# anon-aadhaar/anon-aadhaar-halo2

Hardware: AMD Instinct MI355X
Metric: create_proof wall-clock (ms) + proofs/sec, full Aadhaar circuit, 1/2/4/8 GPU (higher is better)
Workload: dtype u32 limbs (254-bit Montgomery integers: 9 x 29-bit in the hot products, 8 x 32-bit elsewhere)

## Files before the change

### anon-aadhaar-halo2_amd/csrc/msm.hip

```cpp
#include <stdlib.h>
#include <string.h>

#include "common.hpp"
#include "fp29.cuh"
#include "fp29_quad.cuh"

using namespace bn254;

struct amdzk_srs {
  uint32_t k = 0;
  uint32_t c = 0;
  uint32_t W = 0;
  size_t n = 0;
  G1Affine* table[AMDZK_NUM_BASES] = {nullptr, nullptr, nullptr};
  G1Affine* base[AMDZK_NUM_BASES] = {nullptr, nullptr, nullptr};
  std::mutex prefix_guard;
  double prefix_build_ms = 0;
};
static size_t srs_basis_bytes(const amdzk_srs* s) { return ((size_t)s->W + 1) * s->n * sizeof(G1Affine); }

uint32_t zk_srs_k(const amdzk_srs* srs) { return srs->k; }
bool zk_srs_has_basis(const amdzk_srs* srs, int basis) { return srs && basis >= 0 && basis < AMDZK_NUM_BASES && srs->table[basis]; }

namespace {
// ... 1305 lines not shown
  ZK_LAUNCH(ctx, "msm_blk_offsets", msm_blk_offsets_kernel, dim3((nb + 255) / 256, (unsigned)ncols), dim3(256), 0, blk_hist, cnt, nb, g.nblk);
  ZK_LAUNCH(ctx, "msm_scan", msm_scan_kernel, dim3((unsigned)ncols), dim3(1024), scan_shmem, cnt, off[0], nb, 1u, 1);
  if (per_window) ZK_TRY(launch_digits_win<true>(ctx, g.c, da, dgrid));
  else if (d_col_ptrs) ZK_TRY((launch_digits<true, true>(ctx, g.c, da, dgrid, g.big_digits)));
  else ZK_TRY((launch_digits<true, false>(ctx, g.c, da, dgrid, g.big_digits)));
  for (int l = 1; l <= MSM_NLEV; l++) {
    const uint32_t T = l == 1 ? g.T1 : g.TL;
    ZK_LAUNCH(ctx, "msm_scan", msm_scan_kernel, dim3((unsigned)ncols), dim3(1024), scan_shmem, off[l - 1], off[l], nb, T, 2);
    AccArgs a;
    a.off_in = off[l - 1];
    a.off_out = off[l];
    a.nb = nb;
    a.T = T;
    a.entries = entries;
    a.ecap = g.ecap;
    a.table = table;
    a.in_list = list[l - 1];
    a.in_cap = g.cap[l - 1];
    a.out_list = list[l];
    a.out_cap = g.cap[l];
    const size_t threads = (g.cap[l - 1] + T - 1) / T;
    dim3 grid((unsigned)((threads + MSM_THREADS - 1) / MSM_THREADS), (unsigned)ncols);
    if (l == 1) {
      ZK_LAUNCH(ctx, "msm_accum_l1", msm_accum_seg_kernel<true>, grid, dim3(MSM_THREADS), 0, a);
      ZK_HIP(ctx, hipEventRecord(l1_done, ctx->stream));
    } else if (quad_on && !(getenv("AMDZK_FOLD_QUAD") && atoi(getenv("AMDZK_FOLD_QUAD")) == 0)) {
      const dim3 qgrid((unsigned)((4 * threads + MSM_THREADS - 1) / MSM_THREADS), (unsigned)ncols);
      ZK_LAUNCH(ctx, "msm_accum_fold", msm_accum_fold_quad_kernel, qgrid, dim3(MSM_THREADS), 0, a);
    } else {
      ZK_LAUNCH(ctx, "msm_accum_fold", msm_accum_seg_kernel<false>, grid, dim3(MSM_THREADS), 0, a);
    }
  }
  const unsigned fold_w = (unsigned)((g.G + 63) / 64);
  ZK_LAUNCH(ctx, "msm_accum_final", msm_accum_final_kernel, dim3(nb / 64, (unsigned)ncols), dim3(64), 0, off[MSM_NLEV], nb, list[MSM_NLEV],
            g.cap[MSM_NLEV], dense);
  static const int tail_tree = getenv("AMDZK_TAIL_TREE") ? atoi(getenv("AMDZK_TAIL_TREE")) : -1;
  const bool quad = quad_on && fold_w == 1;
  if (quad)
    ZK_LAUNCH(ctx, "msm_rowcol", msm_rowcol_quad_kernel, dim3(64, 2, (unsigned)ncols), dim3(256), 0, dense, nb, rows, cols);
  else if ((tail_tree < 0 ? g.latency : tail_tree != 0) && ncols <= 65535)
    ZK_LAUNCH(ctx, "msm_rowcol", msm_rowcol_tree_kernel, dim3(64, (unsigned)(2 * ((g.G + 63) / 64)), (unsigned)ncols), dim3(64), 0, dense, nb, rows, cols);
  else
    ZK_LAUNCH(ctx, "msm_rowcol", msm_rowcol_kernel, dim3((unsigned)(2 * ((g.G + 63) / 64)), (unsigned)ncols), dim3(64 * ROWCOL_WAVES), 0, dense, nb, rows, cols);
  if (quad) ZK_LAUNCH(ctx, "msm_fold", msm_fold_quad_kernel, dim3((unsigned)ncols), dim3(512), 0, rows, cols, nb, outp);
  else if (fold_w == 1) ZK_LAUNCH(ctx, "msm_fold", msm_fold_kernel<1>, dim3((unsigned)ncols), dim3(128), 0, rows, cols, nb, outp);
  else ZK_LAUNCH(ctx, "msm_fold", msm_fold_kernel<8>, dim3((unsigned)ncols), dim3(64 * (fold_w + 1)), 0, rows, cols, nb, outp);
  return AMDZK_OK;
}

static int msm_check_basis(amdzk_ctx* ctx, const amdzk_srs* srs, int basis) {
  if (!srs || basis < 0 || basis >= AMDZK_NUM_BASES) ZK_FAIL(ctx, AMDZK_E_INVALID, "msm: no parameters or basis %d unknown", basis);
  if (srs->table[basis]) return AMDZK_OK;
  if (basis == AMDZK_BASIS_G_LAGRANGE_PREFIX)
    ZK_FAIL(ctx, AMDZK_E_INVALID, "msm: the prefix-sum basis has not been built (it is made with the first proving key that has permutation columns)");
  ZK_FAIL(ctx, AMDZK_E_INVALID, "msm: basis %d not uploaded", basis);
}

int zk_msm_dev_xyzz(amdzk_ctx* ctx, const amdzk_srs* srs, int basis, const Fr* d_scalars, size_t ncols,
                    size_t len, size_t col_stride, G1X** d_out) {
  ZK_TRY(msm_check_basis(ctx, srs, basis));
  if (len > srs->n) ZK_FAIL(ctx, AMDZK_E_INVALID, "msm: len %zu > 2^k = %zu", len, srs->n);
  if (ncols == 0 || ncols > 65535) ZK_FAIL(ctx, AMDZK_E_INVALID, "msm: ncols %zu out of range", ncols);
  if ((uint64_t)srs->W * srs->n >= (1ull << 31)) ZK_FAIL(ctx, AMDZK_E_UNSUPPORTED, "msm: table too large for 31-bit ids");
  const MsmGeom g = msm_geometry(srs, ncols, len, ctx->msm_latency_mode);
  const size_t o_out = align_up(g.bytes, 256);
  char* ws = nullptr;
  ZK_TRY(zk_ws_reserve(ctx, 1, o_out + align_up(ncols * sizeof(G1X), 256), (void**)&ws));
  G1X* outp = (G1X*)(ws + o_out);
  if (!ctx->msm_l1_evt) ZK_HIP(ctx, hipEventCreateWithFlags(&ctx->msm_l1_evt, hipEventDisableTiming));
  ZK_TRY(msm_group(ctx, srs->table[basis], (uint32_t)srs->n, false, g, ws, d_scalars, ncols, len, col_stride, outp, ctx->msm_l1_evt));
  ctx->msm_l1_fresh = true;
  *d_out = outp;
  return AMDZK_OK;
}

static constexpr size_t MSM_COLS_WS_BYTES = (size_t)16 << 30;
int zk_msm_dev_xyzz_cols(amdzk_ctx* ctx, const amdzk_srs* srs, int basis, const Fr* const* d_col_ptrs, size_t ncols, size_t len,
                         size_t max_ws_bytes, G1X** d_out) {
  ZK_TRY(msm_check_basis(ctx, srs, basis));
  if (len > srs->n) ZK_FAIL(ctx, AMDZK_E_INVALID, "msm: len %zu > 2^k = %zu", len, srs->n);
  if (!d_col_ptrs || ncols == 0) ZK_FAIL(ctx, AMDZK_E_INVALID, "msm: no column pointer table or ncols == 0");
  if ((uint64_t)srs->W * srs->n >= (1ull << 31)) ZK_FAIL(ctx, AMDZK_E_UNSUPPORTED, "msm: table too large for 31-bit ids");
  const size_t cap = max_ws_bytes ? max_ws_bytes : MSM_COLS_WS_BYTES;
  size_t runs = (ncols + 65534) / 65535, per = 0, bytes = 0;
  for (;; runs++) {
    per = (ncols + runs - 1) / runs;
    const size_t last = ncols - (ncols - 1) / per * per;
    bytes = std::max(msm_geometry(srs, per, len, ctx->msm_latency_mode).bytes, msm_geometry(srs, last, len, ctx->msm_latency_mode).bytes);
    if (per == 1 || bytes <= cap) break;
  }
  const size_t o_scratch = align_up(ncols * sizeof(G1X), 256);
  char* ws = nullptr;
  ZK_TRY(zk_ws_reserve(ctx, 1, o_scratch + align_up(bytes, 256), (void**)&ws));
  G1X* outp = (G1X*)ws;
  if (!ctx->msm_l1_evt) ZK_HIP(ctx, hipEventCreateWithFlags(&ctx->msm_l1_evt, hipEventDisableTiming));
  for (size_t first = 0; first < ncols; first += per) {
    const size_t cnt = std::min(per, ncols - first);
    const MsmGeom gr = msm_geometry(srs, cnt, len, ctx->msm_latency_mode);
    ZK_TRY(msm_group(ctx, srs->table[basis], (uint32_t)srs->n, false, gr, ws + o_scratch, nullptr, cnt, len, 0, outp + first, ctx->msm_l1_evt,
                     d_col_ptrs + first));
  }
  ctx->msm_l1_fresh = true;
  *d_out = outp;
  return AMDZK_OK;
}

static uint32_t pick_window_bits_bases(size_t len) {
// ... 103 lines not shown
```

### anon-aadhaar-halo2_amd/csrc/plonk_kernels.hip

```cpp
#include <stdlib.h>
#include <string.h>

#include "plonk_kernels.hpp"
#include "fp29.cuh"

using namespace bn254;

namespace {

__device__ __forceinline__ Fr ld_fr(const Fr* p) {
  const uint4* q = reinterpret_cast<const uint4*>(p);
  uint4 a = q[0], b = q[1];
  Fr r;
  r.l[0] = a.x; r.l[1] = a.y; r.l[2] = a.z; r.l[3] = a.w;
  r.l[4] = b.x; r.l[5] = b.y; r.l[6] = b.z; r.l[7] = b.w;
  return r;
}
__device__ __forceinline__ void st_fr(Fr* p, const Fr& v) {
  uint4* q = reinterpret_cast<uint4*>(p);
  q[0] = make_uint4(v.l[0], v.l[1], v.l[2], v.l[3]);
  q[1] = make_uint4(v.l[4], v.l[5], v.l[6], v.l[7]);
}

__device__ __forceinline__ bool op_reads_col(uint32_t op) {
// ... 297 lines not shown
__global__ __launch_bounds__(256) void batch_invert_kernel(Fr* a, Fr* scratch, size_t total) {
  __shared__ Fr pre[256], suf[256];
  const uint32_t t = threadIdx.x;
  const size_t base = (size_t)blockIdx.x * 256 * BI_E + t;
  Fr acc = Fr::one();
#pragma unroll 1
  for (uint32_t j = 0; j < BI_E; j++) {
    const size_t i = base + (size_t)j * 256;
    if (i >= total) break;
    st_fr(scratch + i, acc);
    const Fr v = ld_fr(a + i);
    if (!v.is_zero()) acc = fr29_mul_std(acc, v);
  }
  pre[t] = acc;
  suf[t] = acc;
  __syncthreads();
  for (uint32_t d = 1; d < 256; d <<= 1) {
    const Fr p = t >= d ? pre[t - d] : Fr::one();
    const Fr q = t + d < 256 ? suf[t + d] : Fr::one();
    __syncthreads();
    if (t >= d) pre[t] = fr29_mul_std(p, pre[t]);
    if (t + d < 256) suf[t] = fr29_mul_std(suf[t], q);
    __syncthreads();
  }
  __shared__ Fr tot_inv;
  if (t == 0) tot_inv = inv_gcd(pre[255]);
  __syncthreads();
  acc = tot_inv;
  if (t > 0) acc = fr29_mul_std(acc, pre[t - 1]);
  if (t < 255) acc = fr29_mul_std(acc, suf[t + 1]);
#pragma unroll 1
  for (uint32_t j = BI_E; j-- > 0;) {
    const size_t i = base + (size_t)j * 256;
    if (i >= total) continue;
    const Fr v = ld_fr(a + i);
    if (v.is_zero()) continue;
    st_fr(a + i, fr29_mul_std(acc, ld_fr(scratch + i)));
    acc = fr29_mul_std(acc, v);
  }
}

__global__ __launch_bounds__(256) void mul_elem_kernel(Fr* a, const Fr* b, size_t total) {
  for (size_t i = (size_t)blockIdx.x * blockDim.x + threadIdx.x; i < total; i += (size_t)gridDim.x * blockDim.x)
    st_fr(a + i, fr29_mul_std(ld_fr(a + i), ld_fr(b + i)));
}

__global__ __launch_bounds__(256) void row_diff_kernel(const Fr* z, Fr* d, size_t n, size_t z_stride, size_t d_stride) {
  const size_t i = (size_t)blockIdx.x * blockDim.x + threadIdx.x;
  if (i >= n) return;
  const Fr* zc = z + (size_t)blockIdx.y * z_stride;
  Fr v = ld_fr(zc + i);
  if (i + 1 < n) v = sub(v, ld_fr(zc + i + 1));
  st_fr(d + (size_t)blockIdx.y * d_stride + i, v);
}

constexpr int SCAN_E = 8;
constexpr int SCAN_BLOCK = 256 * SCAN_E;

__global__ __launch_bounds__(256) void scan_local_kernel(const Fr* in, Fr* out, Fr* totals, size_t n, size_t col_stride,
                                                         uint32_t nblk) {
  __shared__ Fr part[256];
  const uint32_t col = blockIdx.y, blk = blockIdx.x, t = threadIdx.x;
  const Fr* src = in + (size_t)col * col_stride;
  Fr* dst = out + (size_t)col * col_stride;
  const size_t base = (size_t)blk * SCAN_BLOCK + (size_t)t * SCAN_E;
  Fr tot = Fr::one();
#pragma unroll 1
  for (int i = 0; i < SCAN_E; i++)
    if (base + i < n) tot = i == 0 ? ld_fr(src + base) : fr29_mul_std(tot, ld_fr(src + base + i));
  part[t] = tot;
  __syncthreads();
  for (uint32_t d = 1; d < 256; d <<= 1) {
    Fr v = t >= d ? part[t - d] : Fr::one();
    __syncthreads();
    if (t >= d) part[t] = fr29_mul_std(v, part[t]);
    __syncthreads();
  }
  Fr pre = t == 0 ? Fr::one() : part[t - 1];
#pragma unroll 1
  for (int i = 0; i < SCAN_E; i++) {
    if (base + i >= n) break;
    const Fr v = ld_fr(src + base + i);
    st_fr(dst + base + i, pre);
    pre = fr29_mul_std(pre, v);
  }
  if (t == 255) st_fr(totals + (size_t)col * nblk + blk, part[255]);
}

__global__ void scan_blocks_kernel(Fr* totals, const Fr* local, Fr* rel, uint32_t ncols, uint32_t nblk, size_t col_stride,
                                   size_t u) {
  const uint32_t col = blockIdx.x * blockDim.x + threadIdx.x;
  if (col >= ncols) return;
  Fr* t = totals + (size_t)col * nblk;
  Fr acc = Fr::one();
  for (uint32_t b = 0; b < nblk; b++) {
    Fr v = ld_fr(t + b);
    st_fr(t + b, acc);
    acc = fr29_mul_std(acc, v);
  }
  if (rel) st_fr(rel + col, fr29_mul_std(ld_fr(t + u / SCAN_BLOCK), ld_fr(local + (size_t)col * col_stride + u)));
}

__global__ void scan_chain_kernel(const Fr* rel, Fr* start, uint32_t ncols) {
  if (blockIdx.x != 0 || threadIdx.x != 0) return;
  Fr acc = Fr::one();
  for (uint32_t c = 0; c < ncols; c++) {
// ... 400 lines not shown
  for (uint32_t p = 1; p < nparts; p++) acc = add(acc, ld_fr(h + (size_t)p * rows + row));
  st_fr(h + row, acc);
}

int zk_expr_eval_limbs(amdzk_ctx* ctx, const ExprArgs& a, uint32_t depth, const char* name) {
  size_t shmem = (size_t)(depth ? depth : 1) * EXPR_THREADS * 9 * sizeof(uint32_t) + (size_t)17 * EXPR_THREADS * sizeof(uint64_t);
  if (a.nparts > (uint32_t)EXPR_MAX_PARTS) ZK_FAIL(ctx, AMDZK_E_INVALID, "expr_eval_limbs: too many program parts");
  if (a.nparts > 1 && !a.h_out) ZK_FAIL(ctx, AMDZK_E_INVALID, "expr_eval_limbs: a cut program needs h_out (nparts x nrows)");
  const dim3 grid((unsigned)((a.nrows + EXPR_THREADS - 1) / EXPR_THREADS), a.nparts ? a.nparts : 1u), block(EXPR_THREADS);
  if (shmem > 65536) ZK_HIP(ctx, hipFuncSetAttribute((const void*)expr_eval_limbs_kernel, hipFuncAttributeMaxDynamicSharedMemorySize, (int)shmem));
  ZK_LAUNCH(ctx, name, expr_eval_limbs_kernel, grid, block, shmem, a);
  if (a.nparts > 1)
    ZK_LAUNCH(ctx, "sum_parts", sum_parts_kernel, dim3((unsigned)((a.nrows + 255) / 256)), dim3(256), 0, a.h_out, a.nrows, a.nparts);
  return AMDZK_OK;
}

int zk_chacha20_fr_random(amdzk_ctx* ctx, Fr* d_out, size_t n, const uint32_t key[8], uint64_t counter0, const Fr& r3) {
  ChaChaKey k;
  memcpy(k.k, key, sizeof(k.k));
  if (n) ZK_LAUNCH(ctx, "chacha20_fr_random", chacha20_fr_random_kernel, dim3((unsigned)((n + 255) / 256)), dim3(256), 0, d_out, n, k, counter0, r3);
  return AMDZK_OK;
}

int zk_chacha20_blind_rows(amdzk_ctx* ctx, Fr* d_cols, size_t col_stride, size_t row0, uint32_t cnt, uint32_t ncols, const uint32_t key[8],
                           uint64_t counter0, uint32_t draw_stride, const Fr& r3) {
  ChaChaKey k;
  memcpy(k.k, key, sizeof(k.k));
  const size_t total = (size_t)cnt * ncols;
  if (total) ZK_LAUNCH(ctx, "chacha20_blind_rows", chacha20_blind_rows_kernel, dim3((unsigned)((total + 255) / 256)), dim3(256), 0, d_cols + row0, total, k,
                       counter0, r3, cnt, draw_stride, col_stride);
  return AMDZK_OK;
}

int zk_batch_invert(amdzk_ctx* ctx, Fr* d_a, Fr* d_scratch, size_t total) {
  const size_t per_wg = (size_t)256 * BI_E;
  if (total) ZK_LAUNCH(ctx, "batch_invert", batch_invert_kernel, dim3((unsigned)((total + per_wg - 1) / per_wg)), dim3(256), 0, d_a, d_scratch, total);
  return AMDZK_OK;
}

int zk_mul_elem(amdzk_ctx* ctx, Fr* d_a, const Fr* d_b, size_t total) {
  unsigned gx = (unsigned)((total + 255) / 256);
  if (gx > 4096) gx = 4096;
  if (total) ZK_LAUNCH(ctx, "mul_elem", mul_elem_kernel, dim3(gx), dim3(256), 0, d_a, d_b, total);
  return AMDZK_OK;
}

int zk_row_diff(amdzk_ctx* ctx, const Fr* d_z, Fr* d_d, size_t ncols, size_t n, size_t z_stride, size_t d_stride) {
  if (ncols == 0 || n == 0) return AMDZK_OK;
  if (ncols > 65535) ZK_FAIL(ctx, AMDZK_E_INVALID, "row_diff: %zu columns > 65535", ncols);
  ZK_LAUNCH(ctx, "row_diff", row_diff_kernel, dim3((unsigned)((n + 255) / 256), (unsigned)ncols), dim3(256), 0, d_z, d_d, n, z_stride, d_stride);
  return AMDZK_OK;
}

size_t zk_scan_totals_elems(size_t n, size_t ncols) { return ((n + SCAN_BLOCK - 1) / SCAN_BLOCK) * ncols; }

int zk_running_product(amdzk_ctx* ctx, Fr* d_cols, size_t ncols, size_t n, size_t col_stride, bool chain, size_t u, Fr* d_tmp) {
  if (ncols == 0) return AMDZK_OK;
  const uint32_t nblk = (uint32_t)((n + SCAN_BLOCK - 1) / SCAN_BLOCK);
  Fr* totals = d_tmp;
  Fr* rel = totals + (size_t)nblk * ncols;
  Fr* start = rel + ncols;
  ZK_LAUNCH(ctx, "scan_local", scan_local_kernel, dim3(nblk, (unsigned)ncols), dim3(256), 0, d_cols, d_cols, totals, n, col_stride, nblk);
  ZK_LAUNCH(ctx, "scan_blocks", scan_blocks_kernel, dim3((unsigned)((ncols + 63) / 64)), dim3(64), 0, totals, d_cols,
            chain ? rel : (Fr*)nullptr, (uint32_t)ncols, nblk, col_stride, u);
  if (chain) ZK_LAUNCH(ctx, "scan_chain", scan_chain_kernel, dim3(1), dim3(64), 0, rel, start, (uint32_t)ncols);
  unsigned gx = (unsigned)((n + 255) / 256);
  if (gx > 1024) gx = 1024;
  ZK_LAUNCH(ctx, "scan_apply", scan_apply_kernel, dim3(gx, (unsigned)ncols), dim3(256), 0, d_cols, totals, chain ? start : (const Fr*)nullptr, n,
            col_stride, nblk);
  return AMDZK_OK;
}

int zk_poly_eval(amdzk_ctx* ctx, const Fr* const* d_polys, const Fr* d_points, Fr* d_out, size_t nq, uint32_t n) {
  if (!nq) return AMDZK_OK;
  const uint32_t nseg = (n + 65535u) / 65536u;
  if (nseg <= 1 || nq > 65535) {
    ZK_LAUNCH(ctx, "poly_eval", poly_eval_kernel, dim3((unsigned)nq), dim3(256), 0, d_polys, d_points, d_out, n, (Fr*)nullptr);
    return AMDZK_OK;
  }
  Fr* parts = nullptr;
  ZK_TRY(zk_ws_reserve(ctx, 4, nq * nseg * sizeof(Fr), (void**)&parts));
  ZK_LAUNCH(ctx, "poly_eval", poly_eval_kernel, dim3((unsigned)nq, nseg), dim3(256), 0, d_polys, d_points, d_out, n, parts);
  ZK_LAUNCH(ctx, "poly_eval_combine", poly_eval_combine_kernel, dim3((unsigned)((nq + 63) / 64)), dim3(64), 0, (const Fr*)parts, d_points, d_out, (uint32_t)nq,
            nseg);
  return AMDZK_OK;
}

int zk_lincomb(amdzk_ctx* ctx, const Fr* const* d_polys, const Fr* d_coefs, uint32_t m, Fr* d_out, size_t n, bool accumulate) {
  if (m == 0) {
    if (!accumulate && n) ZK_HIP(ctx, hipMemsetAsync(d_out, 0, n * sizeof(Fr), ctx->stream));
    return AMDZK_OK;
  }
  unsigned gx = (unsigned)((n + 255) / 256);
  if (gx > 2048) gx = 2048;
  uint32_t nparts = 1;
  while (nparts < 16 && (size_t)gx * nparts * 2 <= 2048 && m / (nparts * 2) >= 32) nparts *= 2;
  if (nparts == 1) {
    ZK_LAUNCH(ctx, "lincomb", lincomb_kernel, dim3(gx), dim3(256), 0, d_polys, d_coefs, m, d_out, n, accumulate ? 1 : 0, m, (size_t)0);
    return AMDZK_OK;
  }
  Fr* parts = nullptr;
  ZK_TRY(zk_ws_reserve(ctx, 4, (size_t)nparts * n * sizeof(Fr), (void**)&parts));
  const uint32_t per_part = (m + nparts - 1) / nparts;
  ZK_LAUNCH(ctx, "lincomb", lincomb_kernel, dim3(gx, nparts), dim3(256), 0, d_polys, d_coefs, m, parts, n, 0, per_part, n);
  ZK_LAUNCH(ctx, "lincomb_sum_parts", lincomb_sum_parts_kernel, dim3(gx), dim3(256), 0, (const Fr*)parts, n, nparts, d_out, n, accumulate ? 1 : 0);
  return AMDZK_OK;
// ... 175 lines not shown
```

### anon-aadhaar-halo2_amd/csrc/plonk_kernels.hpp

```cpp
#pragma once
#include "common.hpp"

constexpr int EXPR_THREADS = 128;

enum ExprOp : uint32_t {
  OP_END = 0,
  OP_PUSH_COL = 1,
  OP_PUSH_CONST = 2,
  OP_ADD = 3,
  OP_SUB = 4,
  OP_MUL = 5,
  OP_NEG = 6,
  OP_MUL_CONST = 7,
  OP_ADD_CONST = 8,
  OP_MUL_COL = 9,
  OP_ADD_COL = 10,
  OP_SUB_COL = 11,
  OP_ACC = 12,
  OP_STORE = 13,
  OP_SQR = 14,
  OP_PUSH_HOT = 15,
  OP_MUL_HOT = 16,
  OP_REDUCE = 17,
  OP_SUB_BIG = 18,
  OP_NEG_BIG = 19,
  OP_WACC = 20,
  OP_WFLUSH = 21,
  OP_PICK = 22,
  OP_NIP = 23,
};

constexpr int EXPR_HOT = 4;
constexpr int EXPR_MAX_PARTS = 8;
constexpr uint32_t EXPR_NO_SLOT = 0xffffffffu;

struct ExprInstr {
  uint32_t op_arg;
  int32_t rot;
  const bn254::Fr* ptr;
};

struct ExprArgs {
  const ExprInstr* prog;
  uint32_t prog_len;
  const bn254::Fr* const* cols;
  bn254::Fr* const* outs;
  bn254::Fr* h_out;
  size_t mask;
  size_t nrows;
  uint32_t hot[EXPR_HOT];
  uint32_t radix261;
  uint32_t nparts;
  uint32_t part_start[EXPR_MAX_PARTS], part_len[EXPR_MAX_PARTS];
};

int zk_expr_eval(amdzk_ctx* ctx, const ExprArgs& a, uint32_t depth, const char* name);
int zk_expr_eval_limbs(amdzk_ctx* ctx, const ExprArgs& a, uint32_t depth, const char* name);
int zk_chacha20_fr_random(amdzk_ctx* ctx, bn254::Fr* d_out, size_t n, const uint32_t key[8], uint64_t counter0, const bn254::Fr& r3);
int zk_chacha20_blind_rows(amdzk_ctx* ctx, bn254::Fr* d_cols, size_t col_stride, size_t row0, uint32_t cnt, uint32_t ncols, const uint32_t key[8],
                           uint64_t counter0, uint32_t draw_stride, const bn254::Fr& r3);
int zk_batch_invert(amdzk_ctx* ctx, bn254::Fr* d_a, bn254::Fr* d_scratch, size_t total);
int zk_mul_elem(amdzk_ctx* ctx, bn254::Fr* d_a, const bn254::Fr* d_b, size_t total);
int zk_row_diff(amdzk_ctx* ctx, const bn254::Fr* d_z, bn254::Fr* d_d, size_t ncols, size_t n, size_t z_stride, size_t d_stride);
size_t zk_scan_totals_elems(size_t n, size_t ncols);
int zk_running_product(amdzk_ctx* ctx, bn254::Fr* d_cols, size_t ncols, size_t n, size_t col_stride, bool chain, size_t u,
                       bn254::Fr* d_tmp);
int zk_poly_eval(amdzk_ctx* ctx, const bn254::Fr* const* d_polys, const bn254::Fr* d_points, bn254::Fr* d_out, size_t nq, uint32_t n);
int zk_lincomb(amdzk_ctx* ctx, const bn254::Fr* const* d_polys, const bn254::Fr* d_coefs, uint32_t m, bn254::Fr* d_out, size_t n,
               bool accumulate);
int zk_scale(amdzk_ctx* ctx, bn254::Fr* d_a, size_t n, const bn254::Fr& c);
int zk_sub_low(amdzk_ctx* ctx, bn254::Fr* d_a, const bn254::Fr* d_low, uint32_t m);
int zk_kate_div(amdzk_ctx* ctx, bn254::Fr* const* d_polys, const bn254::Fr* d_roots, size_t npolys, uint32_t n);
int zk_kate_div_from(amdzk_ctx* ctx, bn254::Fr* const* d_polys, const bn254::Fr* const* d_srcs, const bn254::Fr* d_roots, const bn254::Fr* d_lows,
                     uint32_t low_stride, size_t npolys, uint32_t n);
int zk_scatter_rows(amdzk_ctx* ctx, bn254::Fr* d_dst, size_t col_stride, size_t row0, const bn254::Fr* d_src, uint32_t cnt,
                    uint32_t ncols);
int zk_sort_keys(amdzk_ctx* ctx, bn254::Fr* d_cols, size_t ncols, uint32_t n, size_t col_stride);
int zk_sort_keys2(amdzk_ctx* ctx, bn254::Fr* d_cols, size_t ncols_a, bn254::Fr* d_cols_b, size_t ncols_b, uint32_t n, size_t col_stride);
int zk_lookup_permute(amdzk_ctx* ctx, bn254::Fr* A, bn254::Fr* Ts, bn254::Fr* S, bn254::Fr* left, size_t L, uint32_t n, uint32_t u,
                      uint32_t* flags, size_t flag_stride, int* d_err, size_t tables_presorted = 0);
```

### anon-aadhaar-halo2_amd/csrc/prover.hip

```cpp
#include <stdlib.h>
#include <string.h>

#include <algorithm>
#include <array>
#include <chrono>
#include <map>
#include <memory>
#include <string>

#include "hostcrypto.hpp"
#include "pkblob.hpp"
#include "check_kernels.hpp"
#include "plonk_kernels.hpp"

using namespace bn254;
using zkhost::Blake2bWrite;
using zkhost::ChaCha20Rng;

struct amdzk_srs;
struct amdzk_domain;
int zk_msm_dev_xyzz(amdzk_ctx* ctx, const amdzk_srs* srs, int basis, const Fr* d_scalars, size_t ncols, size_t len, size_t col_stride,
                    G1X** d_out);
int zk_msm_dev_xyzz_cols(amdzk_ctx* ctx, const amdzk_srs* srs, int basis, const Fr* const* d_col_ptrs, size_t ncols, size_t len,
                         size_t max_ws_bytes, G1X** d_out);
// ... 757 lines not shown
  if (!getenv("AMDZK_TRACE")) return;
  uint8_t b[32];
  zkhost::fr_to_repr(v, b);
  fprintf(stderr, "[amdzk] %s ", label);
  for (int i = 31; i >= 0; i--) fprintf(stderr, "%02x", b[i]);
  fprintf(stderr, "\n");
}
void trace_pt(const char* label, const G1Affine& p) {
  if (!getenv("AMDZK_TRACE")) return;
  uint8_t b[32];
  zkhost::fq_to_repr(p.x, b);
  fprintf(stderr, "[amdzk] %s x=", label);
  for (int i = 31; i >= 0; i--) fprintf(stderr, "%02x", b[i]);
  fprintf(stderr, "\n");
}

}

static int quotient_from_cosets(amdzk_ctx* ctx, amdzk_pk* pk) {
  ZK_TRY(upload_consts261(ctx, pk));
  ZK_TRY(upload_ypow(ctx, pk));
  if (!pk->h_terms) ZK_HIP(ctx, hipMemsetAsync(pk->hq, 0, (size_t)pk->ext * 32, ctx->stream));
  ZK_TRY(run_program(ctx, pk, pk->prog_h, true, nullptr, pk->hq, "expr_evaluate_h"));
  ZK_TRY(zk_cosets_to_pieces(ctx, pk->dom, pk->hq, pk->hpieces, pk->qdeg));
  return AMDZK_OK;
}
static int quotient_pieces(amdzk_ctx* ctx, amdzk_pk* pk) {
  ZK_TRY(zk_coeff_to_cosets_r261(ctx, pk->dom, pk->PQ, pk->n, pk->PC, pk->ext, pk->NP));
  return quotient_from_cosets(ctx, pk);
}

static int alloc_proof_workspace(amdzk_ctx* ctx, amdzk_pk* pk) {
  const size_t n = pk->n, ext = pk->ext;
  const uint32_t A = pk->A, I = pk->I, L = pk->L, ns = pk->nsets;
#define KG_TRY(x) ZK_TRY(x)
  pk->NP = (size_t)A + I + 2 * L + ns + L;
  KG_TRY(dalloc(ctx, pk, &pk->P, pk->NP * n));
  KG_TRY(dalloc(ctx, pk, &pk->PQ, pk->NP * n));
  KG_TRY(dalloc(ctx, pk, &pk->PC, pk->NP * ext));
  KG_TRY(dalloc(ctx, pk, &pk->ci, (size_t)L * n));
  KG_TRY(dalloc(ctx, pk, &pk->ct, (size_t)L * n));
  KG_TRY(dalloc(ctx, pk, &pk->lk_ts, (size_t)L * n));
  KG_TRY(dalloc(ctx, pk, &pk->lk_left, (size_t)L * n));
  KG_TRY(dalloc(ctx, pk, &pk->lk_flags, (size_t)4 * L * (n + 8)));
  KG_TRY(dalloc(ctx, pk, &pk->d_err, 1));
  KG_TRY(dalloc(ctx, pk, &pk->rnd, n));
  KG_TRY(dalloc(ctx, pk, &pk->hq, (size_t)H_PARTS_MAX * ext));
  KG_TRY(dalloc(ctx, pk, &pk->hpieces, (size_t)pk->qdeg * n));
  KG_TRY(dalloc(ctx, pk, &pk->hpoly, n));
  const size_t nfrac = std::max<size_t>(std::max<size_t>(ns, L), 1);
  KG_TRY(dalloc(ctx, pk, &pk->frac, nfrac * n));
  KG_TRY(dalloc(ctx, pk, &pk->scratch, std::max(nfrac * n, ext)));
  KG_TRY(dalloc(ctx, pk, &pk->scan_tmp, zk_scan_totals_elems(n, nfrac) + 2 * nfrac + 8));
  KG_TRY(dalloc(ctx, pk, &pk->frac2, std::max<size_t>(L, 1) * n));
  KG_TRY(dalloc(ctx, pk, &pk->scratch2, std::max<size_t>(L, 1) * n));
  KG_TRY(dalloc(ctx, pk, &pk->scan_tmp2, zk_scan_totals_elems(n, std::max<size_t>(L, 1)) + 2 * std::max<size_t>(L, 1) + 8));
  const size_t max_rsets = pk->max_sets;
  KG_TRY(dalloc(ctx, pk, &pk->sets_L, max_rsets * n));
  KG_TRY(dalloc(ctx, pk, &pk->sets_N, max_rsets * n));
  KG_TRY(dalloc(ctx, pk, &pk->hx, n));
  pk->small_cap = std::max<size_t>((size_t)pk->NP * (pk->bf + 2) + 4096, 8192);
  for (int l = 0; l < 3; l++) KG_TRY(dalloc(ctx, pk, &pk->small_l[l], pk->small_cap));
  pk->small = pk->small_l[0];
  pk->pin_cap = std::max<size_t>((size_t)8 << 20, 2 * n * 32);
  if (hipHostMalloc((void**)&pk->pin, pk->pin_cap + 64, hipHostMallocDefault) != hipSuccess) {
    pk->pin = nullptr;
    pk->pin_cap = 0;
    ZK_FAIL(ctx, AMDZK_E_NOMEM, "prover: hipHostMalloc of the pinned staging area failed");
  }
  pk->h_err = (int*)(pk->pin + pk->pin_cap);
  pk->ptrs_cap = 8192;
  for (int l = 0; l < 3; l++) {
    void** pp = nullptr;
    KG_TRY(dalloc(ctx, pk, &pp, pk->ptrs_cap));
    pk->ptrs_l[l] = pp;
  }
  pk->ptrs = pk->ptrs_l[0];

#undef KG_TRY
  return AMDZK_OK;
}

static int build_column_tables(amdzk_ctx* ctx, amdzk_pk* pk) {
  const size_t n = pk->n, ext = pk->ext;
  const uint32_t F = pk->F, A = pk->A, I = pk->I, S = pk->S, L = pk->L, ns = pk->nsets;
#define KG_TRY(x) ZK_TRY(x)
  {
    std::vector<const Fr*> lag(pk->nslots_lag()), ex(pk->nslots_ext());
    for (uint32_t i = 0; i < F; i++) lag[pk->sl_fixed(i)] = pk->fixed_lag + (size_t)i * n, ex[i] = pk->fixed_coset + (size_t)i * ext;
    for (uint32_t i = 0; i < A; i++) lag[pk->sl_adv(i)] = pk->adv() + (size_t)i * n, ex[pk->sl_adv(i)] = pk->PC + (size_t)i * ext;
    for (uint32_t i = 0; i < I; i++) lag[pk->sl_inst(i)] = pk->inst() + (size_t)i * n, ex[pk->sl_inst(i)] = pk->PC + (size_t)(A + i) * ext;
    for (uint32_t i = 0; i < S; i++) lag[pk->sl_sigma(i)] = pk->sigma_lag + (size_t)i * n, ex[pk->se_sigma(i)] = pk->sigma_coset + (size_t)i * ext;
    for (uint32_t i = 0; i < S; i++) lag[pk->sl_dxw(i)] = pk->dxw_lag + (size_t)i * n, ex[pk->se_dx(i)] = pk->dx_coset + (size_t)i * ext;
    for (uint32_t l = 0; l < L; l++) {
      lag[pk->sl_ci(l)] = pk->ci + (size_t)l * n;
      lag[pk->sl_ct(l)] = pk->ct + (size_t)l * n;
      lag[pk->sl_la(l)] = pk->la() + (size_t)l * n;
      lag[pk->sl_ls(l)] = pk->ls() + (size_t)l * n;
      ex[pk->se_la(l)] = pk->PC + (size_t)(A + I + l) * ext;
      ex[pk->se_ls(l)] = pk->PC + (size_t)(A + I + L + l) * ext;
      ex[pk->se_zl(l)] = pk->PC + (size_t)(A + I + 2 * L + ns + l) * ext;
    }
    for (uint32_t s = 0; s < ns; s++) ex[pk->se_zp(s)] = pk->PC + (size_t)(A + I + 2 * L + s) * ext;
    lag[pk->sl_omega()] = pk->omega_pow;
    ex[pk->se_l0()] = pk->l0_c;
    ex[pk->se_llast()] = pk->llast_c;
    ex[pk->se_lactive()] = pk->lactive_c;
// ... 1010 lines not shown
          ZK_TRY(put_challenge(i, chal[i]));
        }
      before += in_phase;
    }
    ZK_TRY(commit_end(cm_rnd));
    tick("advice (phased)");
    return AMDZK_OK;
  }
  int advice(const void* const* d_advice_all, size_t advice_stride) {
    if (pk->phased()) return advice_phased(d_advice_all, advice_stride);
    for (size_t ci = 0; ci < NC; ci++) {
      ZK_TRY(advice_enqueue(ci, d_advice_all ? d_advice_all[ci] : nullptr, advice_stride));
      ZK_TRY(commit_end(cm_adv));
      ZK_TRY(advice_write());
    }
    ZK_TRY(commit_end(cm_rnd));
    tick("advice");
    return AMDZK_OK;
  }
  int advice_enqueue(size_t ci, const void* d_advice, size_t advice_stride) {
    amdzk_pk* const pk = pks[ci];
    if (A) {
      ZK_HIP(ctx, hipMemcpy2DAsync(pk->adv(), n * 32, d_advice, advice_stride * 32, n * 32, A, hipMemcpyDeviceToDevice, ctx->stream));
      ZK_TRY(blind(M, pk->adv(), A, usable, bf + 1, draws.advice(ci), draws.col));
    }
    cm_adv = Commit();
    if (A && !serial) ZK_TRY(commit_begin(M, AMDZK_BASIS_G_LAGRANGE, pk->adv(), A, cm_adv));
    ZK_TRY(transforms_on_B(pk, M, 0, (size_t)A + I, cm_adv.begun));
    if (A && !cm_adv.begun) ZK_TRY(commit_begin(M, AMDZK_BASIS_G_LAGRANGE, pk->adv(), A, cm_adv));
    return AMDZK_OK;
  }
  int advice_write() { return write_points(cm_adv.pts, "advice"); }
  int lookups() {
    for (size_t ci = 0; ci < NC && L; ci++) {
      ZK_TRY(lookups_enqueue(ci));
      ZK_TRY(commit_end(cm_lk));
      ZK_TRY(lookups_write(ci));
    }
    tick("lookups_permuted");
    return AMDZK_OK;
  }
  int lookups_enqueue(size_t ci) {
    if (!L) return AMDZK_OK;
    amdzk_pk* const pk = pks[ci];
    ZK_TRY(run_program(ctx, pk, pk->prog_compress, false, pk->d_outs_compress, nullptr, "expr_lookup_compress"));
    ZK_TRY(d2d(ctx, pk->la(), pk->ci, (size_t)L * n * 32));
    ZK_TRY(zk_permute_expression_pairs(ctx, pk->la(), pk->ct, pk->lk_ts, pk->ls(), pk->lk_left, pk->lk_flags, pk->d_err, L, (uint32_t)n,
                                       (uint32_t)usable, pk->lk_ts_const, pk->lk_const));
    *pk->h_err = 0;
    ZK_HIP(ctx, hipMemcpyAsync(pk->h_err, pk->d_err, sizeof(int), hipMemcpyDeviceToHost, ctx->stream));
    tick("  lookup: device permute");
    ZK_TRY(blind(M, pk->la(), L, usable, bf + 1, draws.lookup(ci), draws.lk_col));
    ZK_TRY(blind(M, pk->ls(), L, usable, bf + 1, draws.lookup(ci) + draws.col, draws.lk_col));
    cm_lk = Commit();
    if (!serial) ZK_TRY(commit_begin(M, AMDZK_BASIS_G_LAGRANGE, pk->la(), 2 * L, cm_lk));
    ZK_TRY(transforms_on_B(pk, M, (size_t)A + I, 2 * (size_t)L, cm_lk.begun));
    if (!cm_lk.begun) ZK_TRY(commit_begin(M, AMDZK_BASIS_G_LAGRANGE, pk->la(), 2 * L, cm_lk));
    return AMDZK_OK;
  }
  int lookups_write(size_t ci) {
    if (!L) return AMDZK_OK;
    amdzk_pk* const pk = pks[ci];
    if (*pk->h_err) ZK_FAIL(ctx, AMDZK_E_INVALID, "create_proof: lookup %d input not in table (ConstraintSystemFailure)", *pk->h_err - 1);
    const std::vector<G1Affine>& cm = cm_lk.pts;
    for (uint32_t l = 0; l < L; l++) {
      std::vector<G1Affine> two = {cm[l], cm[L + l]};
      ZK_TRY(write_points(two, "lookup_permuted"));
    }
    return AMDZK_OK;
  }
  int lookup_products(size_t ci, bool ordered_behind_m) {
    amdzk_pk* const pk = pks[ci];
    if (!ordered_behind_m) ZK_TRY(zk_stream_after(C, M));
    ZK_TRY(on_lane(C, run_program(C, pk, pk->prog_lfrac, false, pk->d_outs_lfrac, nullptr, "expr_lookup_fractions")));
    ZK_TRY(on_lane(C, zk_batch_invert(C, pk->frac2, pk->scratch2, (size_t)L * n)));
    ZK_TRY(on_lane(C, zk_mul_elem(C, pk->zl(), pk->frac2, (size_t)L * n)));
    ZK_TRY(on_lane(C, zk_running_product(C, pk->zl(), L, n, n, false, 0, pk->scan_tmp2)));
    ZK_TRY(blind(C, pk->zl(), L, n - bf, bf, draws.lookup_product(ci), draws.col));
    if (serial) ZK_TRY(transforms_on_B(pk, C, (size_t)A + I + 2 * L + ns, L));
    ZK_TRY(commit_begin(C, AMDZK_BASIS_G_LAGRANGE, pk->zl(), L, cm_zl[ci]));
    if (!serial) ZK_TRY(transforms_on_B(pk, C, (size_t)A + I + 2 * L + ns, L, true));
    return AMDZK_OK;
  }
  int perm_products(size_t ci) {
    amdzk_pk* const pk = pks[ci];
    ZK_TRY(run_program(ctx, pk, pk->prog_pfrac, false, pk->d_outs_pfrac, nullptr, "expr_perm_fractions"));
    tick("  perm: fractions program");
    ZK_TRY(zk_batch_invert(ctx, pk->frac, pk->scratch, (size_t)ns * n));
    tick("  perm: batch invert");
    ZK_TRY(zk_mul_elem(ctx, pk->zp(), pk->frac, (size_t)ns * n));
    ZK_TRY(zk_running_product(ctx, pk->zp(), ns, n, n, true, usable, pk->scan_tmp));
    tick("  perm: running product");
    ZK_TRY(blind(M, pk->zp(), ns, n - bf, bf, draws.perm_product(ci), draws.col));
    return zk_row_diff(M, pk->zp(), pk->frac, ns, n, n, n);
  }
  int perm_commit(size_t ci) {
    amdzk_pk* const pk = pks[ci];
    if (serial) ZK_TRY(transforms_on_B(pk, M, (size_t)A + I + 2 * L, ns));
    return commit_begin(M, AMDZK_BASIS_G_LAGRANGE_PREFIX, pk->frac, ns, cm_zp[ci]);
  }
  int products() {
    if (!serial) {
      if (L) ZK_TRY(zk_stream_after(C, M));
      if (ns) ZK_TRY(perm_products(0));
      if (L) ZK_TRY(lookup_products(0, true));
      if (ns) ZK_TRY(perm_commit(0));
    } else {
      ZK_TRY(products_enqueue_serial());
    }
    if (ns && !serial) ZK_TRY(transforms_on_B(pk, M, (size_t)A + I + 2 * L, ns, true));
    return products_write();
  }
  int products_enqueue_serial() {
    for (size_t ci = 0; ci < NC && L; ci++) ZK_TRY(lookup_products(ci, false));
    for (size_t ci = 0; ci < NC && ns; ci++) {
      ZK_TRY(perm_products(ci));
      ZK_TRY(perm_commit(ci));
// ... 169 lines not shown
    if (2 * nq > pk->ptrs_cap || nq * (maxm + 2) > pk->small_cap) ZK_FAIL(ctx, AMDZK_E_NOMEM, "create_proof: too many opening points");
    void** pt = (void**)pk->ptrs;
    ZK_TRY(h2d_staged(ctx, pk, pt, q_dst.data(), nq * sizeof(Fr*)));
    ZK_TRY(h2d_staged(ctx, pk, pt + nq, q_src.data(), nq * sizeof(Fr*)));
    ZK_TRY(upload_small_on(M, q_root, 0));
    ZK_TRY(upload_small_on(M, q_low, nq));
    ZK_TRY(upload_small_on(M, q_coef, nq + q_low.size()));
    ZK_TRY(zk_kate_div_from(ctx, (Fr* const*)pt, (const Fr* const*)(pt + nq), pk->small, pk->small + nq, (uint32_t)maxm, nq, (uint32_t)n));
    ZK_TRY(zk_lincomb(ctx, (const Fr* const*)pt, pk->small + nq + q_low.size(), (uint32_t)nq, pk->hx, n, false));
    return commit_write(AMDZK_BASIS_G, pk->hx, 1, "shplonk_h1");
  }
  int shplonk_final(const Fr& v, const Fr& u) {
    const size_t nr = mo->sets.size();
    std::vector<uint32_t> super(rot_pt.size());
    for (size_t r = 0; r < super.size(); r++) super[r] = (uint32_t)r;
    std::sort(super.begin(), super.end(), [&](uint32_t r1, uint32_t r2) { return fr_less_canon(rot_canon[r1], rot_canon[r2]); });
    Fr zt = Fr::one();
    for (uint32_t r : super) zt = mul(zt, sub(u, rot_pt[r]));
    std::vector<const Fr*> pp(nr + 1);
    std::vector<Fr> cf(nr + 1);
    Fr cur = Fr::one(), z0 = Fr::one(), cterm = Fr::zero();
    for (size_t i = 0; i < nr; i++) {
      Fr zi = Fr::one();
      for (uint32_t r : super)
        if (!std::binary_search(mo->sets[i].rot_ids.begin(), mo->sets[i].rot_ids.end(), r)) zi = mul(zi, sub(u, rot_pt[r]));
      if (i == 0) z0 = zi;
      const Fr ri = eval_small(sh.low[i], u);
      Fr w = mul(cur, zi);
      pp[i] = pk->sets_L + i * n;
      cf[i] = w;
      cterm = add(cterm, mul(w, ri));
      cur = mul(cur, v);
    }
    pp[nr] = pk->hx;
    cf[nr] = neg(zt);
    const Fr z0inv = inv(z0);
    for (auto& c : cf) c = mul(c, z0inv);
    cterm = mul(cterm, z0inv);
    Fr* lx = pk->sets_Q;
    ZK_TRY(lincomb(M, pp, cf, lx, n, {cterm, u}));
    std::vector<Fr*> one_p = {lx};
    ZK_TRY(h2d_staged(ctx, pk, (void**)pk->ptrs + nr + 1, one_p.data(), sizeof(Fr*)));
    ZK_TRY(zk_kate_div_from(ctx, (Fr* const*)((void**)pk->ptrs + nr + 1), nullptr, pk->small + nr + 2, pk->small + nr + 1, 1, 1, (uint32_t)n));
    return commit_write(AMDZK_BASIS_G, lx, 1, "shplonk_h2");
  }
};

struct ProofExtras {
  const amdzk_transcript* transcript = nullptr;
  amdzk_phase_fn phase_fn = nullptr;
  void* phase_user = nullptr;
};

int create_proof_body(amdzk_ctx* ctx, amdzk_pk* const* pks, size_t NC, const uint64_t* const* const* instances_all,
                      const size_t* const* instance_lens_all, const void* const* d_advice_all, size_t advice_stride, const RandomSource& rng,
                      int transcript_kind, uint8_t* proof_out, size_t proof_cap, size_t* proof_len, const ProofExtras& ex) {
  amdzk_pk* const pk = pks[0];
  if (!proof_len) ZK_FAIL(ctx, AMDZK_E_INVALID, "create_proof: null argument");
  for (size_t c = 0; c < NC; c++) {
    if (!pks[c] || (pk->A && (!d_advice_all || !d_advice_all[c]))) ZK_FAIL(ctx, AMDZK_E_INVALID, "create_proof: null argument (circuit %zu)", c);
    const amdzk_pk* root_c = pks[c]->clone_of ? pks[c]->clone_of : pks[c];
    const amdzk_pk* root_0 = pk->clone_of ? pk->clone_of : pk;
    if (root_c != root_0) ZK_FAIL(ctx, AMDZK_E_INVALID, "create_proof: circuit %zu's key is not the first key or a workspace clone of it", c);
    for (size_t d = 0; d < c; d++)
      if (pks[d] == pks[c]) ZK_FAIL(ctx, AMDZK_E_INVALID, "create_proof: circuits %zu and %zu share one workspace", d, c);
  }
  if (advice_stride < pk->n) ZK_FAIL(ctx, AMDZK_E_INVALID, "create_proof: advice stride < n");
  if (pk->nphases > 1 && !ex.phase_fn)
    ZK_FAIL(ctx, AMDZK_E_INVALID, "create_proof: the key has advice in %u phases: amdzk_create_proof_opts with a phase callback is needed", pk->nphases);
  const bool use_gwc = (transcript_kind & AMDZK_MULTIOPEN_GWC) != 0;
  transcript_kind &= ~AMDZK_MULTIOPEN_GWC;
  zkhost::Blake2bWrite t_blake;
  zkhost::Keccak256Write t_keccak;
  if (!ex.transcript && transcript_kind != AMDZK_TRANSCRIPT_BLAKE2B && transcript_kind != AMDZK_TRANSCRIPT_KECCAK256_EVM)
    ZK_FAIL(ctx, AMDZK_E_INVALID, "create_proof: unknown transcript kind %d", transcript_kind);
  if (ex.transcript && (!ex.transcript->common_point || !ex.transcript->common_scalar || !ex.transcript->write_point ||
                        !ex.transcript->write_scalar || !ex.transcript->squeeze_challenge))
    ZK_FAIL(ctx, AMDZK_E_INVALID, "create_proof: amdzk_transcript has a null member");
  const amdzk_transcript no_transcript = {};
  zkhost::CallbackWrite t_caller(ex.transcript ? *ex.transcript : no_transcript);
  zkhost::TranscriptWrite& T = ex.transcript                                  ? (zkhost::TranscriptWrite&)t_caller
                               : transcript_kind == AMDZK_TRANSCRIPT_BLAKE2B ? (zkhost::TranscriptWrite&)t_blake
                                                                             : (zkhost::TranscriptWrite&)t_keccak;
#define T_OK()                                                                                                   \
  do {                                                                                                           \
    if (T.failed) ZK_FAIL(ctx, AMDZK_E_INVALID, "create_proof: the caller's transcript reported an error");     \
  } while (0)
  amdzk_ctx *B = ctx, *C = ctx;
  if (pk->use_lanes && NC == 1) {
    ZK_TRY(zk_lane(ctx, 0, &B));
    ZK_TRY(zk_lane(ctx, 1, &C));
  }
  const bool serial = B == ctx;
  struct LatencyMode {
    amdzk_ctx* c[3];
    bool keep[3];
    LatencyMode(amdzk_ctx* m, amdzk_ctx* b, amdzk_ctx* cc, bool on) : c{m, b, cc} {
      for (int i = 0; i < 3; i++) keep[i] = c[i]->msm_latency_mode, c[i]->msm_latency_mode = on || keep[i];
    }
    ~LatencyMode() {
      for (int i = 0; i < 3; i++) c[i]->msm_latency_mode = keep[i];
    }
  } latency_mode(ctx, B, C, !serial && !(getenv("AMDZK_LATENCY_MODE") && atoi(getenv("AMDZK_LATENCY_MODE")) == 0));

  Prover P(ctx, pks, NC, B, C, T, rng);
  P.phase_fn = ex.phase_fn;
  P.phase_user = ex.phase_user;
  ZK_TRY(P.instances(instances_all, instance_lens_all));
  T_OK();
  ZK_TRY(P.random_poly());
  ZK_TRY(P.advice(d_advice_all, advice_stride));
  T_OK();
  const Fr theta = P.challenge("theta");
  ZK_TRY(P.put_consts({{&amdzk_pk::c_theta, theta}}));
  ZK_TRY(P.lookups());
  const Fr beta = P.challenge("beta");
  const Fr gamma = P.challenge("gamma");
  T_OK();
  if (pk->S && beta.is_zero()) ZK_FAIL(ctx, AMDZK_E_UNSUPPORTED, "create_proof: the challenge beta is zero (probability 2^-254): the factored permutation terms need 1 / beta");
  ZK_TRY(P.put_consts({{&amdzk_pk::c_beta, beta}, {&amdzk_pk::c_gamma, gamma}, {&amdzk_pk::c_betainv, inv(beta)}}));
  P.tick("  perm: challenges+consts");
  ZK_TRY(P.products());
// ... 342 lines not shown
                            uint8_t* proof_out, size_t proof_cap, size_t* proof_len) {
  ZK_ENTER(ctx);
  if (!ctx) return AMDZK_E_INVALID;
  if (!pks || n_circuits == 0 || !pks[0]) ZK_FAIL(ctx, AMDZK_E_INVALID, "create_proof_opts: no circuits");
  if (!opts) ZK_FAIL(ctx, AMDZK_E_INVALID, "create_proof_opts: null options");
  if (opts->size < sizeof(amdzk_proof_opts))
    ZK_FAIL(ctx, AMDZK_E_INVALID, "create_proof_opts: amdzk_proof_opts.size is %zu, this library needs %zu", opts->size, sizeof(amdzk_proof_opts));
  RandomSource rs;
  if (opts->scalars) {
    const size_t need = DrawLayout(pks[0], n_circuits).total;
    if (opts->scalar_count < need) ZK_FAIL(ctx, AMDZK_E_INVALID, "create_proof_opts: %zu scalars given, %zu needed", opts->scalar_count, need);
    rs.scalars = opts->scalars;
  } else {
    rs = RandomSource(opts->rng_seed);
  }
  ProofExtras ex;
  ex.transcript = opts->transcript;
  ex.phase_fn = opts->phase_fn;
  ex.phase_user = opts->phase_user;
  return create_proof_impl(ctx, pks, n_circuits, instances, instance_lens, d_advice, advice_stride, rs, opts->transcript_kind, proof_out, proof_cap,
                           proof_len, ex);
}

static int proof_batch(amdzk_ctx* ctx, amdzk_pk* const* pks, size_t n_proofs, const uint64_t* const* const* instances,
                       const size_t* const* instance_lens, const void* const* d_advice, size_t advice_stride, const amdzk_batch_opts* opts,
                       uint8_t* proofs_out, size_t proof_stride, size_t* proof_lens, int* statuses, bool* ran) {
  if (!pks || n_proofs == 0) ZK_FAIL(ctx, AMDZK_E_INVALID, "create_proof_batch: no proofs");
  if (!opts || !proofs_out || !proof_lens) ZK_FAIL(ctx, AMDZK_E_INVALID, "create_proof_batch: null argument");
  if (opts->size < sizeof(amdzk_batch_opts))
    ZK_FAIL(ctx, AMDZK_E_INVALID, "create_proof_batch: amdzk_batch_opts.size is %zu, this library needs %zu", opts->size, sizeof(amdzk_batch_opts));
  if (!opts->rng_seeds && !opts->scalars) ZK_FAIL(ctx, AMDZK_E_INVALID, "create_proof_batch: neither rng_seeds nor scalars");
  for (size_t b = 0; b < n_proofs; b++) {
    if (!pks[b]) ZK_FAIL(ctx, AMDZK_E_INVALID, "create_proof_batch: null key (proof %zu)", b);
    const amdzk_pk* root_b = pks[b]->clone_of ? pks[b]->clone_of : pks[b];
    const amdzk_pk* root_0 = pks[0]->clone_of ? pks[0]->clone_of : pks[0];
    if (root_b != root_0) ZK_FAIL(ctx, AMDZK_E_INVALID, "create_proof_batch: proof %zu's key is not the first key or a workspace clone of it", b);
    for (size_t d = 0; d < b; d++)
      if (pks[d] == pks[b]) ZK_FAIL(ctx, AMDZK_E_INVALID, "create_proof_batch: proofs %zu and %zu share one workspace", d, b);
    if (pks[0]->A && (!d_advice || !d_advice[b])) ZK_FAIL(ctx, AMDZK_E_INVALID, "create_proof_batch: null advice (proof %zu)", b);
    if (opts->scalars && !opts->scalars[b]) ZK_FAIL(ctx, AMDZK_E_INVALID, "create_proof_batch: null scalars (proof %zu)", b);
  }
  amdzk_pk* const pk = pks[0];
  if (pk->phased())
    ZK_FAIL(ctx, AMDZK_E_UNSUPPORTED, "create_proof_batch: the key has challenge phases or challenges: prove it with amdzk_create_proof_opts");
  if (advice_stride < pk->n) ZK_FAIL(ctx, AMDZK_E_INVALID, "create_proof_batch: advice stride < n");
  const bool use_gwc = (opts->transcript_kind & AMDZK_MULTIOPEN_GWC) != 0;
  const int kind = opts->transcript_kind & ~AMDZK_MULTIOPEN_GWC;
  if (kind != AMDZK_TRANSCRIPT_BLAKE2B && kind != AMDZK_TRANSCRIPT_KECCAK256_EVM)
    ZK_FAIL(ctx, AMDZK_E_INVALID, "create_proof_batch: unknown transcript kind %d", kind);
  const size_t psize = amdzk_proof_size(pk, opts->transcript_kind);
  if (proof_stride < psize) ZK_FAIL(ctx, AMDZK_E_INVALID, "create_proof_batch: proof_stride %zu < proof size %zu", proof_stride, psize);
  if (opts->scalars && opts->scalar_count < DrawLayout(pk, 1).total)
    ZK_FAIL(ctx, AMDZK_E_INVALID, "create_proof_batch: %zu scalars given, %zu needed", opts->scalar_count, DrawLayout(pk, 1).total);

  *ran = true;
  Gang g(ctx);
  for (size_t b = 0; b < n_proofs; b++) {
    std::unique_ptr<Gang::Member> m(new Gang::Member);
    m->index = b;
    m->pk = pks[b];
    if (opts->scalars) m->rng.scalars = opts->scalars[b];
    else m->rng = RandomSource(opts->rng_seeds[b]);
    zkhost::TranscriptWrite& T = kind == AMDZK_TRANSCRIPT_BLAKE2B ? (zkhost::TranscriptWrite&)m->t_blake : (zkhost::TranscriptWrite&)m->t_keccak;
    m->P.reset(new Prover(ctx, &pks[b], 1, ctx, ctx, T, m->rng));
    m->P->sink = &m->deferred;
    g.members.push_back(std::move(m));
  }
  const int run = g.run(instances, instance_lens, d_advice, advice_stride, use_gwc);
  int first = AMDZK_OK;
  std::string first_err;
  for (auto& m : g.members) {
    if (m->live && run != AMDZK_OK) {
      m->live = false;
      m->status = run;
      m->err = ctx->err;
    }
    if (m->live && m->T().proof.size() > proof_stride) {
      m->live = false;
      m->status = AMDZK_E_INVALID;
      m->err = "proof " + std::to_string(m->index) + ": create_proof: proof buffer too small";
    }
    if (statuses) statuses[m->index] = m->status;
    proof_lens[m->index] = m->live ? m->T().proof.size() : 0;
    if (m->live) memcpy(proofs_out + m->index * proof_stride, m->T().proof.data(), m->T().proof.size());
    else if (first == AMDZK_OK) first = m->status, first_err = m->err;
  }
  if (first != AMDZK_OK) {
    (void)zk_sync_all(ctx);
    ctx->err = first_err;
  }
  return first;
}
int amdzk_create_proof_batch(amdzk_ctx* ctx, amdzk_pk* const* pks, size_t n_proofs, const uint64_t* const* const* instances,
                             const size_t* const* instance_lens, const void* const* d_advice, size_t advice_stride,
                             const amdzk_batch_opts* opts, uint8_t* proofs_out, size_t proof_stride, size_t* proof_lens, int* statuses) {
  ZK_ENTER(ctx);
  if (!ctx) return AMDZK_E_INVALID;
  bool ran = false;
  const int r = proof_batch(ctx, pks, n_proofs, instances, instance_lens, d_advice, advice_stride, opts, proofs_out, proof_stride, proof_lens,
                            statuses, &ran);
  if (!ran)
    for (size_t b = 0; b < n_proofs; b++) {
      if (statuses) statuses[b] = r;
      if (proof_lens) proof_lens[b] = 0;
    }
  return r;
// ... 389 lines not shown
```

Measured before the change: 98.44.

## Commit permuted lookup columns via prefix-sum basis on row differences

Lookup permuted input/table columns are now committed against the prefix-sum Lagrange basis using forward row differences (next minus current), then the committed points are negated on the host to recover the true commitment. Permuted lookup columns are sorted and hold many repeated values, so their differences are mostly zero, which makes the MSM sparse and cheaper. This adds a difference kernel, doubles the frac2 buffer, and forces the prefix basis to be built for keys that have lookups, at the cost of extra memory and a one-time basis build.

After: 99.49, median of 6. +1.1%, better.

```diff
diff --git a/anon-aadhaar-halo2_amd/csrc/msm.hip b/anon-aadhaar-halo2_amd/csrc/msm.hip
--- a/anon-aadhaar-halo2_amd/csrc/msm.hip
+++ b/anon-aadhaar-halo2_amd/csrc/msm.hip
@@ -1381,7 +1381,7 @@
   if (!srs || basis < 0 || basis >= AMDZK_NUM_BASES) ZK_FAIL(ctx, AMDZK_E_INVALID, "msm: no parameters or basis %d unknown", basis);
   if (srs->table[basis]) return AMDZK_OK;
   if (basis == AMDZK_BASIS_G_LAGRANGE_PREFIX)
-    ZK_FAIL(ctx, AMDZK_E_INVALID, "msm: the prefix-sum basis has not been built (it is made with the first proving key that has permutation columns)");
+    ZK_FAIL(ctx, AMDZK_E_INVALID, "msm: the prefix-sum basis has not been built (it is made with the first proving key that has permutation columns or lookups)");
   ZK_FAIL(ctx, AMDZK_E_INVALID, "msm: basis %d not uploaded", basis);
 }
 
diff --git a/anon-aadhaar-halo2_amd/csrc/plonk_kernels.hip b/anon-aadhaar-halo2_amd/csrc/plonk_kernels.hip
--- a/anon-aadhaar-halo2_amd/csrc/plonk_kernels.hip
+++ b/anon-aadhaar-halo2_amd/csrc/plonk_kernels.hip
@@ -373,6 +373,15 @@
   Fr v = ld_fr(zc + i);
   if (i + 1 < n) v = sub(v, ld_fr(zc + i + 1));
   st_fr(d + (size_t)blockIdx.y * d_stride + i, v);
+}
+
+__global__ __launch_bounds__(256) void row_diff_next_kernel(const Fr* a, Fr* e, size_t n, size_t a_stride, size_t e_stride) {
+  const size_t i = (size_t)blockIdx.x * blockDim.x + threadIdx.x;
+  if (i >= n) return;
+  const Fr* ac = a + (size_t)blockIdx.y * a_stride;
+  const Fr cur = ld_fr(ac + i);
+  const Fr v = i + 1 < n ? sub(ld_fr(ac + i + 1), cur) : neg(cur);
+  st_fr(e + (size_t)blockIdx.y * e_stride + i, v);
 }
 
 constexpr int SCAN_E = 8;
@@ -879,6 +888,13 @@
   return AMDZK_OK;
 }
 
+int zk_row_diff_next(amdzk_ctx* ctx, const Fr* d_a, Fr* d_e, size_t ncols, size_t n, size_t a_stride, size_t e_stride) {
+  if (ncols == 0 || n == 0) return AMDZK_OK;
+  if (ncols > 65535) ZK_FAIL(ctx, AMDZK_E_INVALID, "row_diff_next: %zu columns > 65535", ncols);
+  ZK_LAUNCH(ctx, "row_diff_next", row_diff_next_kernel, dim3((unsigned)((n + 255) / 256), (unsigned)ncols), dim3(256), 0, d_a, d_e, n, a_stride, e_stride);
+  return AMDZK_OK;
+}
+
 size_t zk_scan_totals_elems(size_t n, size_t ncols) { return ((n + SCAN_BLOCK - 1) / SCAN_BLOCK) * ncols; }
 
 int zk_running_product(amdzk_ctx* ctx, Fr* d_cols, size_t ncols, size_t n, size_t col_stride, bool chain, size_t u, Fr* d_tmp) {
diff --git a/anon-aadhaar-halo2_amd/csrc/plonk_kernels.hpp b/anon-aadhaar-halo2_amd/csrc/plonk_kernels.hpp
--- a/anon-aadhaar-halo2_amd/csrc/plonk_kernels.hpp
+++ b/anon-aadhaar-halo2_amd/csrc/plonk_kernels.hpp
@@ -62,6 +62,7 @@
 int zk_batch_invert(amdzk_ctx* ctx, bn254::Fr* d_a, bn254::Fr* d_scratch, size_t total);
 int zk_mul_elem(amdzk_ctx* ctx, bn254::Fr* d_a, const bn254::Fr* d_b, size_t total);
 int zk_row_diff(amdzk_ctx* ctx, const bn254::Fr* d_z, bn254::Fr* d_d, size_t ncols, size_t n, size_t z_stride, size_t d_stride);
+int zk_row_diff_next(amdzk_ctx* ctx, const bn254::Fr* d_a, bn254::Fr* d_e, size_t ncols, size_t n, size_t a_stride, size_t e_stride);
 size_t zk_scan_totals_elems(size_t n, size_t ncols);
 int zk_running_product(amdzk_ctx* ctx, bn254::Fr* d_cols, size_t ncols, size_t n, size_t col_stride, bool chain, size_t u,
                        bn254::Fr* d_tmp);
diff --git a/anon-aadhaar-halo2_amd/csrc/prover.hip b/anon-aadhaar-halo2_amd/csrc/prover.hip
--- a/anon-aadhaar-halo2_amd/csrc/prover.hip
+++ b/anon-aadhaar-halo2_amd/csrc/prover.hip
@@ -833,7 +833,7 @@
   KG_TRY(dalloc(ctx, pk, &pk->frac, nfrac * n));
   KG_TRY(dalloc(ctx, pk, &pk->scratch, std::max(nfrac * n, ext)));
   KG_TRY(dalloc(ctx, pk, &pk->scan_tmp, zk_scan_totals_elems(n, nfrac) + 2 * nfrac + 8));
-  KG_TRY(dalloc(ctx, pk, &pk->frac2, std::max<size_t>(L, 1) * n));
+  KG_TRY(dalloc(ctx, pk, &pk->frac2, std::max<size_t>(2 * (size_t)L, 1) * n));
   KG_TRY(dalloc(ctx, pk, &pk->scratch2, std::max<size_t>(L, 1) * n));
   KG_TRY(dalloc(ctx, pk, &pk->scan_tmp2, zk_scan_totals_elems(n, std::max<size_t>(L, 1)) + 2 * std::max<size_t>(L, 1) + 8));
   const size_t max_rsets = pk->max_sets;
@@ -1950,17 +1950,20 @@
     tick("  lookup: device permute");
     ZK_TRY(blind(M, pk->la(), L, usable, bf + 1, draws.lookup(ci), draws.lk_col));
     ZK_TRY(blind(M, pk->ls(), L, usable, bf + 1, draws.lookup(ci) + draws.col, draws.lk_col));
+    ZK_TRY(zk_row_diff_next(M, pk->la(), pk->frac2, 2 * (size_t)L, n, n, n));
     cm_lk = Commit();
-    if (!serial) ZK_TRY(commit_begin(M, AMDZK_BASIS_G_LAGRANGE, pk->la(), 2 * L, cm_lk));
+    if (!serial) ZK_TRY(commit_begin(M, AMDZK_BASIS_G_LAGRANGE_PREFIX, pk->frac2, 2 * L, cm_lk));
     ZK_TRY(transforms_on_B(pk, M, (size_t)A + I, 2 * (size_t)L, cm_lk.begun));
-    if (!cm_lk.begun) ZK_TRY(commit_begin(M, AMDZK_BASIS_G_LAGRANGE, pk->la(), 2 * L, cm_lk));
+    if (!cm_lk.begun) ZK_TRY(commit_begin(M, AMDZK_BASIS_G_LAGRANGE_PREFIX, pk->frac2, 2 * L, cm_lk));
     return AMDZK_OK;
   }
   int lookups_write(size_t ci) {
     if (!L) return AMDZK_OK;
     amdzk_pk* const pk = pks[ci];
     if (*pk->h_err) ZK_FAIL(ctx, AMDZK_E_INVALID, "create_proof: lookup %d input not in table (ConstraintSystemFailure)", *pk->h_err - 1);
-    const std::vector<G1Affine>& cm = cm_lk.pts;
+    std::vector<G1Affine>& cm = cm_lk.pts;
+    for (auto& p : cm)
+      if (!p.y.is_zero()) p.y = neg(p.y);
     for (uint32_t l = 0; l < L; l++) {
       std::vector<G1Affine> two = {cm[l], cm[L + l]};
       ZK_TRY(write_points(two, "lookup_permuted"));
@@ -2236,6 +2239,8 @@
   void* phase_user = nullptr;
 };
 
+int ensure_lookup_basis(amdzk_ctx* ctx, const amdzk_pk* pk) { return pk->L ? zk_srs_ensure_prefix(ctx, pk->srs) : AMDZK_OK; }
+
 int create_proof_body(amdzk_ctx* ctx, amdzk_pk* const* pks, size_t NC, const uint64_t* const* const* instances_all,
                       const size_t* const* instance_lens_all, const void* const* d_advice_all, size_t advice_stride, const RandomSource& rng,
                       int transcript_kind, uint8_t* proof_out, size_t proof_cap, size_t* proof_len, const ProofExtras& ex) {
@@ -2252,6 +2257,7 @@
   if (advice_stride < pk->n) ZK_FAIL(ctx, AMDZK_E_INVALID, "create_proof: advice stride < n");
   if (pk->nphases > 1 && !ex.phase_fn)
     ZK_FAIL(ctx, AMDZK_E_INVALID, "create_proof: the key has advice in %u phases: amdzk_create_proof_opts with a phase callback is needed", pk->nphases);
+  ZK_TRY(ensure_lookup_basis(ctx, pk));
   const bool use_gwc = (transcript_kind & AMDZK_MULTIOPEN_GWC) != 0;
   transcript_kind &= ~AMDZK_MULTIOPEN_GWC;
   zkhost::Blake2bWrite t_blake;
@@ -2700,6 +2706,7 @@
   if (proof_stride < psize) ZK_FAIL(ctx, AMDZK_E_INVALID, "create_proof_batch: proof_stride %zu < proof size %zu", proof_stride, psize);
   if (opts->scalars && opts->scalar_count < DrawLayout(pk, 1).total)
     ZK_FAIL(ctx, AMDZK_E_INVALID, "create_proof_batch: %zu scalars given, %zu needed", opts->scalar_count, DrawLayout(pk, 1).total);
+  ZK_TRY(ensure_lookup_basis(ctx, pk));
 
   *ran = true;
   Gang g(ctx);
```
